# heyblackC/DFMIR

Measured on AMD Instinct MI355X. Metric: train-step image-pairs/sec (fwd+bwd): 2D 256x256 bs=16 and 3D 160^3 bs=1, higher is better.
Workload: dtype f32 (fp16x2-split MFMA, fp32 accumulate)

## Files before the change

### dfmir_amd/csrc/conv3x3s.hip

```cpp
#include "split_f16.h"

#ifndef PP_COMPUTE_PRIO
#define PP_COMPUTE_PRIO 1
#endif
#ifndef CS_COMPUTE_PRIO
#define CS_COMPUTE_PRIO 1
#endif
#ifndef CS_STORE_PRIO
#define CS_STORE_PRIO 0
#endif
typedef __bf16 bf16x8 __attribute__((ext_vector_type(8)));
typedef __bf16 bf16x2 __attribute__((ext_vector_type(2)));
typedef _Float16 f16x2 __attribute__((ext_vector_type(2)));
typedef float f32x2 __attribute__((ext_vector_type(2)));

__device__ __forceinline__ unsigned pk_bf16(float a, float b) {
  const f32x2 v = {a, b};
  return __builtin_bit_cast(unsigned, __builtin_convertvector(v, bf16x2));
}

template <int NSP>
__device__ __forceinline__ void split_pair(float x0, float x1, unsigned (&p)[NSP]) {
  if constexpr (NSP == 3) {
    p[0] = pk_bf16(x0, x1);
// ... 448 lines not shown
          if (k.act == 1) v = v > 0.f ? v : v * k.slope;
          else if (k.act == 2) v = tanhf(v);
          yb[(long long)co * HWo + q] = v;
        }
      }
    }
  }
}

constexpr int CS_TH = 8, CS_TW = 32, CS_PW = CS_TW + 2, CS_XP = 352;

__device__ __forceinline__ void cs_mma_chunk(const u32x4* __restrict__ Ab, const u32x4* __restrict__ Xb, int abase,
                                             const int (&pb)[2], f32x16 (&acc)[4],
                                             const __amdgpu_buffer_rsrc_t rw_, const unsigned (&wb)[9], u32x4 (&rw)[9],
                                             const __amdgpu_buffer_rsrc_t rx_, const unsigned (&gvo)[2][8],
                                             unsigned (&rx)[2][8]) {
  constexpr int SA = 9 * 2 * 64, SX = 2 * CS_XP;
  using P = Prod<2>;
  u32x4 a[2][2][2], b[2][2][2];
#define CS_LOAD(set_, t_)                                                                        \
  {                                                                                              \
    _Pragma("unroll") for (int i = 0; i < 2; ++i)                                                \
      _Pragma("unroll") for (int s = 0; s < 2; ++s) a[set_][i][s] = Ab[s * SA + (t_) * 128 + abase + i * 32]; \
    _Pragma("unroll") for (int j = 0; j < 2; ++j)                                                \
      _Pragma("unroll") for (int s = 0; s < 2; ++s) b[set_][j][s] = Xb[s * SX + pb[j] + ((t_) / 3) * CS_PW + (t_) % 3]; \
  }
  CS_LOAD(0, 0)
  __builtin_amdgcn_sched_barrier(0);
#pragma unroll
  for (int t = 0; t < 9; ++t) {
    if (t < 8) CS_LOAD((t + 1) & 1, t + 1)
#pragma unroll
    for (int q = 0; q < 3; ++q) {
      const int L = 3 * t + q;
      if (L < 9) rw[L] = __builtin_amdgcn_raw_buffer_load_b128(rw_, wb[L], 0, 0);
      else if (L < 25) rx[(L - 9) >> 3][(L - 9) & 7] = __builtin_amdgcn_raw_buffer_load_b32(rx_, gvo[(L - 9) >> 3][(L - 9) & 7], 0, 0);
    }
#pragma unroll
    for (int q = 0; q < P::N; ++q)
#pragma unroll
      for (int i = 0; i < 2; ++i)
#pragma unroll
        for (int j = 0; j < 2; ++j)
          acc[2 * i + j] = mma16<2>(b[t & 1][j][P::B[q]], a[t & 1][i][P::A[q]], acc[2 * i + j]);
    const int nds = t < 8 ? 8 : 0, nvm = (3 * t + 3 <= 25) ? 3 : (25 - 3 * t > 0 ? 25 - 3 * t : 0);
#pragma unroll
    for (int i = 0; i < 12; ++i) {
      __builtin_amdgcn_sched_group_barrier(0x008, 1, 0);
      if (i < nds) __builtin_amdgcn_sched_group_barrier(0x100, 1, 0);
      else if (i - nds < nvm) __builtin_amdgcn_sched_group_barrier(0x020, 1, 0);
    }
    __builtin_amdgcn_sched_barrier(0);
  }
#undef CS_LOAD
}

template <int CPG, int XP, int NW, int NS>
__device__ __forceinline__ void cs_mma_chunk_rr(const u32x4* __restrict__ Ab, const u32x4* __restrict__ Xb, int abase,
                                                int xb, f32x16 (&acc)[4],
                                                const __amdgpu_buffer_rsrc_t rw_, const unsigned (&wb)[NW], u32x4 (&rw)[NW],
                                                const __amdgpu_buffer_rsrc_t rx_, const unsigned (&gvo)[NS][8],
                                                unsigned (&rx)[NS][8]) {
  constexpr int SA = 9 * 2 * CPG, SX = 2 * XP;
  constexpr int NL = NW + 8 * NS;
  using P = Prod<2>;
  u32x4 a[9][2], xr[3][6][2];
#define CS_LDA(st_, s_) a[st_][s_] = Ab[(s_) * SA + (((st_) % 3) * 3 + (st_) / 3) * (2 * CPG) + abase];
#define CS_LDX(kx_, r_, s_) xr[kx_][r_][s_] = Xb[(s_) * SX + xb + (r_) * CS_PW + (kx_)];
#define CS_NEED(n_)                                                                              \
  {                                                                                              \
    constexpr int kx_ = (n_) / 3, ky_ = (n_) % 3;                                                \
    CS_LDA(n_, 1)                                                                                \
    if (ky_ == 0) { _Pragma("unroll") for (int r = 0; r < 4; ++r) CS_LDX(kx_, r, 0) }            \
    else CS_LDX(kx_, ky_ + 3, 0)                                                                 \
    CS_LDA(n_, 0)                                                                                \
    if (ky_ == 0) { _Pragma("unroll") for (int r = 0; r < 4; ++r) CS_LDX(kx_, r, 1) }            \
    else CS_LDX(kx_, ky_ + 3, 1)                                                                 \
  }
  CS_NEED(0)
  __builtin_amdgcn_sched_barrier(0);
#pragma unroll
  for (int st = 0; st < 9; ++st) {
    const int kx = st / 3, ky = st % 3;
    int nds = 0;
    if (st == 0) { CS_NEED(1) CS_NEED(2) nds = 8; }
    else if (st == 1) { CS_NEED(3) nds = 10; }
    else if (st == 2) { CS_NEED(4) nds = 4; }
    else if (st == 3) { CS_NEED(5) nds = 4; }
    else if (st == 4) { CS_NEED(6) nds = 10; }
    else if (st == 5) { CS_NEED(7) nds = 4; }
    else if (st == 6) { CS_NEED(8) nds = 4; }
    int L0, nvm;
    if (NL == 25) {
      L0 = st == 0 ? 0 : st == 1 ? 4 : st == 2 ? 6 : st == 3 ? 10 : st == 4 ? 14 : st == 5 ? 16 : st == 6 ? 20 : 24;
      nvm = (st == 1 || st == 4) ? 2 : (st == 7 ? 1 : (st == 8 ? 0 : 4));
    } else {
      const int lo = NL / 8, ex = NL % 8;
      L0 = st * lo + (st < ex ? st : ex);
      nvm = st < 8 ? lo + (st < ex ? 1 : 0) : 0;
    }
#pragma unroll
    for (int q = 0; q < (NL + 7) / 8; ++q) {
      const int L = L0 + q;
      if (q < nvm) {
        if (L < NW) rw[L] = __builtin_amdgcn_raw_buffer_load_b128(rw_, wb[L], 0, 0);
        else if (L < NL) rx[(L - NW) >> 3][(L - NW) & 7] = __builtin_amdgcn_raw_buffer_load_b32(rx_, gvo[(L - NW) >> 3][(L - NW) & 7], 0, 0);
      }
    }
#pragma unroll
    for (int q = 0; q < P::N; ++q)
#pragma unroll
      for (int j = 0; j < 4; ++j)
        acc[j] = mma16<2>(xr[kx][ky + j][P::B[q]], a[st][P::A[q]], acc[j]);
#pragma unroll
    for (int i = 0; i < 12; ++i) {
      __builtin_amdgcn_sched_group_barrier(0x008, 1, 0);
      if (i < nds) __builtin_amdgcn_sched_group_barrier(0x100, 1, 0);
      if (i >= 12 - nvm) __builtin_amdgcn_sched_group_barrier(0x020, 1, 0);
    }
    __builtin_amdgcn_sched_barrier(0);
  }
#undef CS_NEED
#undef CS_LDA
#undef CS_LDX
}

struct ConvCsP {
  int N, Cin, Cout, Hi, Wi, Ho, Wo, pad, pad_mode, act;
  float slope;
  int tiles_x, tiles_y;
  const float* res;
  const float* ring;
  int ring_rl;
  int xcd_pair;
  int dephase;
  int vec4;
};

#ifdef CS_TRACE
__device__ unsigned g_cs_trace[8 * 32 * 8 + 8];
extern "C" int dfmir_cs_trace_dump(unsigned* out) {
  return (int)hipMemcpyFromSymbol(out, HIP_SYMBOL(g_cs_trace), sizeof(unsigned) * (8 * 32 * 8 + 8));
}
#define TRC(slot_) { if (trace_blk && lane == 0) trc[((grp * 4 + wid) * 32 + (h & 31)) * 8 + (slot_)] = (unsigned)__builtin_readcyclecounter(); }
__device__ unsigned g_cs_wg[2048 * 6];
extern "C" int dfmir_cs_wg_dump(unsigned* out) {
  return (int)hipMemcpyFromSymbol(out, HIP_SYMBOL(g_cs_wg), sizeof(unsigned) * 2048 * 6);
}
#define WGT(slot_) { if (threadIdx.x == 0 && blockIdx.x < 2048 && blockIdx.y == 0) g_cs_wg[blockIdx.x * 6 + (slot_)] = (unsigned)wall_clock64(); }
#else
#define WGT(slot_)
#define TRC(slot_)
#endif
template <bool RR, int CPG, int TH>
__global__ __launch_bounds__(512, 1) void conv3x3_split_cs_k(const float* __restrict__ x, const u32x4* __restrict__ ws,
                                                             const float* __restrict__ bias, float* __restrict__ y,
                                                             ConvCsP k, SplitScale sc) {
  static_assert((CPG == 64 && TH == 8) || (RR && CPG == 32 && TH == 16), "tile forms");
  constexpr int CS_TH = TH;
  constexpr int NSP = 2, XP = (TH == 8 ? CS_XP : 640), NPOS = (CS_TH + 2) * CS_PW;
  constexpr int WUG = NSP * 9 * 2 * CPG;
  constexpr int NW = (WUG + 255) / 256;
  constexpr int NS = (NPOS + 255) / 256;
  __shared__ __attribute__((aligned(16))) u32x4 Wg[2][WUG];
  __shared__ __attribute__((aligned(16))) u32x4 Xs[2][NSP * 2 * XP];
  __shared__ float bs[2 * CPG];
#ifdef CS_TRACE
  __shared__ unsigned trc[8 * 32 * 8];
  const bool trace_blk = blockIdx.x == 300 && blockIdx.y == 0;
  const unsigned long long trc_t0 = __builtin_readcyclecounter(), trc_r0 = wall_clock64();
#endif

  const int grp = __builtin_amdgcn_readfirstlane((int)(threadIdx.x >> 8));
  const int tid = threadIdx.x & 255, lane = tid & 63, wid = tid >> 6;
  const int l31 = lane & 31, lhi = lane >> 5;
  const int HWo = k.Ho * k.Wo, HWi = k.Hi * k.Wi;
  if (k.dephase > 0 && blockIdx.y == 0 && blockIdx.x < 256) {
    const unsigned long long t0 = wall_clock64();
    const unsigned wait = blockIdx.x * (unsigned)k.dephase >> 8;
    while ((unsigned)(wall_clock64() - t0) < wait) __builtin_amdgcn_s_sleep(4);
  }
  WGT(0)
#ifdef CS_TRACE
  if (threadIdx.x == 0 && blockIdx.x < 2048 && blockIdx.y == 0) {
    g_cs_wg[blockIdx.x * 6 + 4] = __builtin_amdgcn_s_getreg(63492);
    g_cs_wg[blockIdx.x * 6 + 5] = __builtin_amdgcn_s_getreg(63508);
  }
#endif
  int bt = blockIdx.x, bm = blockIdx.y;
  if (k.xcd_pair == 1) { bm = (bt >> 3) & 1; bt = ((bt >> 4) << 3) + (bt & 7); }
  else if (k.xcd_pair >= 2) {
    const int ny = k.xcd_pair - 1, per = (int)(gridDim.x >> 3) / ny, j = bt >> 3;
    bm = j % ny;
    bt = (bt & 7) * per + j / ny;
  }
  const int tx = bt % k.tiles_x; bt /= k.tiles_x;
  const int ty = bt % k.tiles_y;
  const int n = bt / k.tiles_y;
  const int oy0 = ty * CS_TH, ox0 = tx * CS_TW;
  const int m0 = bm * (2 * CPG), m0g = m0 + CPG * grp;

  const int ex = scale_exp(reduce_absmax(sc.x_amax, sc.x_n, bs));
  __syncthreads();
  const int ew = (int)sc.w_trailer[1];
  const float xscale = pow2f(ex), oscale = pow2f(-ex), oscale2 = pow2f(-ew);

  constexpr unsigned OOB = 0x80000000u;
  unsigned gvo[NS][8];
#pragma unroll
  for (int s = 0; s < NS; ++s) {
    const int pos = tid + 256 * s;
    int off = -1;
    if (pos < NPOS) {
      const int r = pos / CS_PW, c = pos - r * CS_PW;
      off = halo_offset(oy0 - k.pad + r, ox0 - k.pad + c, k.Hi, k.Wi, k.pad_mode);
    }
#pragma unroll
    for (int c = 0; c < 8; ++c) gvo[s][c] = off < 0 ? OOB : (unsigned)(off + (8 * grp + c) * HWi) * 4u;
  }
  if (threadIdx.x < 2 * CPG) bs[threadIdx.x] = (bias && (m0 + (int)threadIdx.x) < k.Cout) ? bias[m0 + threadIdx.x] : 0.f;

  int pb[2];
#pragma unroll
  for (int j = 0; j < 2; ++j) pb[j] = lhi * XP + (2 * wid + j) * CS_PW + l31;
  const int rowgrp = CPG == 64 ? (wid >> 1) : wid;
  const int xb = lhi * XP + 4 * rowgrp * CS_PW + l31;
  const int abase = lhi * CPG + l31 + ((RR && CPG == 64) ? 32 * (wid & 1) : 0);

  f32x16 acc[4];
#pragma unroll
  for (int i = 0; i < 4; ++i)
#pragma unroll
    for (int r = 0; r < 16; ++r) acc[i][r] = 0.f;

  const float* xn = x + (long long)n * k.Cin * HWi;
  const int chunks8 = (k.Cin + 7) / 8, chunks = (k.Cin + 15) / 16;
  unsigned wb[NW];
#pragma unroll
  for (int j = 0; j < NW; ++j) {
    const int idx = tid + 256 * j;
    const int co = m0g + (idx % CPG), r = idx / CPG;
    const int half = r & 1, st = r >> 1;
    wb[j] = (idx < WUG && co < k.Cout) ? (unsigned)((half * NSP * 9 + st) * k.Cout + co) * 16u : OOB;
  }
  const int wunits8 = NSP * 9 * k.Cout;

  u32x4 rw[NW];
  unsigned rx[NS][8];
#define CS_GLOADW(c_)                                                                            \
  {                                                                                              \
    const int q_ = 2 * (c_);                                                                     \
    const int left_ = chunks8 - q_;                                                              \
    const __amdgpu_buffer_rsrc_t rw_ = __builtin_amdgcn_make_buffer_rsrc(                        \
        const_cast<u32x4*>(ws + (long long)q_ * wunits8), 0,                                     \
        left_ > 0 ? (unsigned)((left_ < 2 ? left_ : 2) * wunits8) * 16u : 0u, 0x00020000);       \
    _Pragma("unroll") for (int j = 0; j < NW; ++j) rw[j] = __builtin_amdgcn_raw_buffer_load_b128(rw_, wb[j], 0, 0); \
  }
#define CS_GLOADX(c_)                                                                            \
  {                                                                                              \
    const int c0_ = 16 * (c_);                                                                   \
    const int left_ = k.Cin - c0_;                                                               \
    const __amdgpu_buffer_rsrc_t rx_ = __builtin_amdgcn_make_buffer_rsrc(                        \
        const_cast<float*>(xn + (long long)c0_ * HWi), 0,                                        \
        left_ > 0 ? (unsigned)((left_ < 16 ? left_ : 16) * HWi) * 4u : 0u, 0x00020000);          \
    _Pragma("unroll") for (int s = 0; s < NS; ++s)                                               \
      _Pragma("unroll") for (int c = 0; c < 8; ++c)                                              \
        rx[s][c] = __builtin_amdgcn_raw_buffer_load_b32(rx_, gvo[s][c], 0, 0);                   \
  }
#define CS_LSTOREW()                                                                             \
  { _Pragma("unroll") for (int j = 0; j < NW; ++j) if (WUG % 256 == 0 || tid + 256 * j < WUG) Wg[grp][tid + 256 * j] = rw[j]; }
#define CS_LSTOREX(buf_)                                                                         \
  {                                                                                              \
    _Pragma("unroll") for (int s = 0; s < NS; ++s) {                                             \
      const int pos = tid + 256 * s;                                                             \
      if (pos < NPOS) {                                                                          \
        float v[8];                                                                              \
        _Pragma("unroll") for (int c = 0; c < 8; ++c) v[c] = __uint_as_float(rx[s][c]);          \
        CS_NORM_PROBE_OPS()                                                                      \
        u32x4 sp[NSP];                                                                           \
        split8_s<NSP>(v, xscale, sp);                                                                      \
        _Pragma("unroll") for (int q = 0; q < NSP; ++q) Xs[buf_][(q * 2 + grp) * XP + pos] = sp[q]; \
      }                                                                                          \
    }                                                                                            \
  }

#ifdef CS_NORM_PROBE
  const float np_r = fmaf(oscale2, 0.f, 1.f), np_m = oscale2 * 0.f, np_lo = fmaf(oscale2, 0.f, -3.0e38f);
#define CS_NORM_PROBE_OPS() _Pragma("unroll") for (int c = 0; c < 8; ++c) v[c] = fmaxf(fmaf(v[c], np_r, np_m), np_lo);
#else
#define CS_NORM_PROBE_OPS()
#endif
  CS_GLOADX(0);
  if (grp == 0) CS_GLOADW(0);
  CS_LSTOREX(0);
  if (grp == 0) CS_LSTOREW();
  if (grp == 1) { CS_GLOADW(0); CS_GLOADX(1); }
  __syncthreads();
  WGT(1)

  for (int h = 0; h < 2 * chunks; ++h) {
    const int c = h >> 1;
    TRC(0)
    if ((h & 1) == grp) {
      __builtin_amdgcn_s_setprio(CS_COMPUTE_PRIO);
      const int qw_ = 2 * (c + 1), lw_ = chunks8 - qw_;
      const __amdgpu_buffer_rsrc_t rwd = __builtin_amdgcn_make_buffer_rsrc(
          const_cast<u32x4*>(ws + (long long)qw_ * wunits8), 0,
          lw_ > 0 ? (unsigned)((lw_ < 2 ? lw_ : 2) * wunits8) * 16u : 0u, 0x00020000);
      const int cx_ = 16 * (c + 1 + grp), lx_ = k.Cin - cx_;
      const __amdgpu_buffer_rsrc_t rxd = __builtin_amdgcn_make_buffer_rsrc(
          const_cast<float*>(xn + (long long)cx_ * HWi), 0,
          lx_ > 0 ? (unsigned)((lx_ < 16 ? lx_ : 16) * HWi) * 4u : 0u, 0x00020000);
      if constexpr (RR) cs_mma_chunk_rr<CPG, XP, NW, NS>(Wg[grp], Xs[c & 1], abase, xb, acc, rwd, wb, rw, rxd, gvo, rx);
      else if constexpr (CPG == 64) cs_mma_chunk(Wg[grp], Xs[c & 1], abase, pb, acc, rwd, wb, rw, rxd, gvo, rx);
    } else {
      __builtin_amdgcn_s_setprio(CS_STORE_PRIO);
      {
#ifdef CS_TRACE
      __builtin_amdgcn_s_waitcnt(0x0f70);
      TRC(3)
#endif
#ifdef CS_TRACE
      CS_LSTOREW();
      TRC(4)
      if (c + 1 < chunks) CS_LSTOREX((c + 1) & 1);
#else
      if (grp == 0) {
        if (c + 1 < chunks) { CS_LSTOREW(); CS_LSTOREX((c + 1) & 1); }
      } else {
        CS_LSTOREW();
        if (c + 1 < chunks) CS_LSTOREX((c + 1) & 1);
      }
#endif
      }
    }
    TRC(1)
#ifndef CS_NO_EARLY_EPI
    if (h + 1 < 2 * chunks)
#endif
    __syncthreads();
    TRC(2)
  }
  WGT(2)
#ifdef CS_TRACE
  if (trace_blk) {
    __syncthreads();
    for (int i = threadIdx.x; i < 8 * 32 * 8; i += 512) g_cs_trace[i] = trc[i];
    if (threadIdx.x == 0) {
      const unsigned long long t1 = __builtin_readcyclecounter(), r1 = wall_clock64();
      g_cs_trace[2048] = (unsigned)trc_t0; g_cs_trace[2049] = (unsigned)t1;
      g_cs_trace[2050] = (unsigned)trc_r0; g_cs_trace[2051] = (unsigned)r1;
    }
  }
#endif
#undef CS_GLOADW
#undef CS_GLOADX
#undef CS_LSTOREW
#undef CS_LSTOREX
#undef CS_NORM_PROBE_OPS

  float* yb = y + (long long)n * k.Cout * HWo;
#pragma unroll
  for (int b = 0; b < 4; ++b) {
    const int i = CPG == 32 ? 0 : (RR ? (wid & 1) : (b >> 1));
    const int row = RR ? 4 * rowgrp + b : 2 * wid + (b & 1);
    const int oy = oy0 + row;
    const int cc = CPG * grp + i * 32 + l31, co = m0 + cc;
#ifdef CS_KO_EPI
    if (oy >= k.Ho || co >= k.Cout || acc[b][0] != 12345.678f) continue;
#else
    if (oy >= k.Ho || co >= k.Cout) continue;
#endif
    const float bv = bs[cc], osc = oscale * oscale2;
    const long long rowoff = (long long)co * HWo + (long long)oy * k.Wo;
    const float* rb = k.res ? k.res + (long long)n * k.Cout * HWo + rowoff : nullptr;
    const float* rg = k.ring ? k.ring + ((long long)n * 4 * k.Cout + co) * k.ring_rl : nullptr;
    const long long ss = (long long)k.Cout * k.ring_rl;
    const bool row_ring = rg != nullptr && (oy == 1 || oy == k.Ho - 2);
    float4 rv[4];
#pragma unroll
    for (int q = 0; q < 4; ++q) {
      rv[q] = make_float4(0.f, 0.f, 0.f, 0.f);
      const int ox = ox0 + 8 * q + 4 * lhi;
      if (rb && ox < k.Wo) {
        if (k.vec4) rv[q] = *reinterpret_cast<const float4*>(rb + ox);
        else {
          rv[q].x = rb[ox];
          if (ox + 1 < k.Wo) rv[q].y = rb[ox + 1];
          if (ox + 2 < k.Wo) rv[q].z = rb[ox + 2];
          if (ox + 3 < k.Wo) rv[q].w = rb[ox + 3];
        }
      }
    }
#pragma unroll
    for (int q = 0; q < 4; ++q) {
      const int ox = ox0 + 8 * q + 4 * lhi;
      if (ox >= k.Wo) continue;
      float v[4];
      const float r4[4] = {rv[q].x, rv[q].y, rv[q].z, rv[q].w};
#pragma unroll
      for (int e = 0; e < 4; ++e) {
        float t = acc[b][4 * q + e] * osc + bv;
        if (k.act == 1) t = t > 0.f ? t : t * k.slope;
        else if (k.act == 2) t = tanhf(t);
        v[e] = t + r4[e];
      }
      if (rg) {
#pragma unroll
        for (int e = 0; e < 4; ++e) {
          const int xx = ox + e;
          if (xx < k.Wo) {
            if (row_ring) {
              if (oy == 1) v[e] += rg[xx + 1] + (xx == 1 ? rg[0] : 0.f) + (xx == k.Wo - 2 ? rg[k.Wo + 1] : 0.f);
              if (oy == k.Ho - 2) v[e] += rg[ss + xx + 1] + (xx == 1 ? rg[ss] : 0.f) + (xx == k.Wo - 2 ? rg[ss + k.Wo + 1] : 0.f);
            }
            if (xx == 1) v[e] += rg[2 * ss + oy + 1];
            if (xx == k.Wo - 2) v[e] += rg[3 * ss + oy + 1];
          }
        }
      }
      float* yp = yb + rowoff + ox;
#ifdef CS_NT_STORE
      if (k.vec4) __builtin_nontemporal_store(f32x4{v[0], v[1], v[2], v[3]}, reinterpret_cast<f32x4*>(yp));
#else
      if (k.vec4) *reinterpret_cast<float4*>(yp) = make_float4(v[0], v[1], v[2], v[3]);
#endif
      else {
        yp[0] = v[0];
        if (ox + 1 < k.Wo) yp[1] = v[1];
        if (ox + 2 < k.Wo) yp[2] = v[2];
        if (ox + 3 < k.Wo) yp[3] = v[3];
      }
    }
  }
#ifdef CS_TRACE
  __builtin_amdgcn_s_waitcnt(0x0f70);
#endif
  WGT(3)
}

#ifdef DFMIR_BUILD_W1
#include "../../scripts/ubench/conv3x3_split_w1.inc"
#endif

static bool cs_plan(const DfConvGeom* g, int* th_out, int* tx_out, int* ty_out) {
  static DfOptFlag nocs_o{"DFMIR_CONV_NO_CS"};
  const bool use_cs = !nocs_o.get();
  static DfOptFlag plain_o{"DFMIR_CONV_CS_PLAIN"};
  const bool rr = !plain_o.get();
  if (!(df_split_mode() == 2 && use_cs && (g->Cout > 64 || rr))) return false;
  const int th = g->Cout > 64 ? 8 : 16;
  const int tx = (g->Wo + CS_TW - 1) / CS_TW, ty = (g->Ho + th - 1) / th;
  const double fill = (double)g->Ho * g->Wo / ((double)tx * CS_TW * ty * th);
  if (!((long long)g->N * tx * ty < (1LL << 31) && fill >= 0.85)) return false;
  *th_out = th; *tx_out = tx; *ty_out = ty;
  return true;
}
static bool split_fwd_geom_ok(const DfConvGeom* g) {
  if (!(g->KD == 1 && g->KH == 3 && g->KW == 3 && g->Di == 1 && g->Do == 1 && g->stride == 1 && g->dil == 1))
    return false;
  if (g->Cout <= 32 || g->Cin < 16 || g->ph != g->pw || g->pd != 0) return false;
  const int p = g->ph;
  if (!(p == 1 || (p == 2 && g->pad_mode == 0))) return false;
  if (g->Ho != g->Hi + 2 * p - 2 || g->Wo != g->Wi + 2 * p - 2) return false;
  const long long HWo = (long long)g->Ho * g->Wo;
  if (HWo >= (1LL << 30) || (long long)g->Hi * g->Wi >= (1LL << 30)) return false;
  if ((long long)((g->Cin + 7) / 8) * 27 * g->Cout * 16 >= (1LL << 31)) return false;
  if (worst_npos(g->Wo, (int)HWo, 128) > 399) return false;
  return true;
}
int df_conv3x3_split_res_ok(const DfConvGeom* g) {
  int th, tx, ty;
  return (df_split_mode() == 2 && split_fwd_geom_ok(g) && cs_plan(g, &th, &tx, &ty)) ? 1 : 0;
}
bool df_conv3x3_split_fwd_try(const DfConvGeom* g, const float* x, const float* x_amax, int x_n, const float* w_packed,
                              const float* bias, const float* res, const float* ring, int ring_rl, float* y,
                              hipStream_t st, int* rc) {
  const int mode = df_split_mode();
  if (mode == 0 || (mode == 2 && !(x_amax && x_n > 0))) return false;
  if (!split_fwd_geom_ok(g)) return false;
  const int p = g->ph;
  const long long HWo = (long long)g->Ho * g->Wo;
  Conv3P k{g->N, g->Cin, g->Cout, g->Hi, g->Wi, g->Ho, g->Wo, p, g->pad_mode, g->act, g->slope, 0};
  const u32x4* ws = reinterpret_cast<const u32x4*>(split_section(w_packed, g->Cin, g->Cout));
  const SplitScale sc{x_amax, x_n, split_trailer(w_packed, g->Cin, g->Cout, mode)};
  static DfOptFlag plain_o{"DFMIR_CONV_CS_PLAIN"};
  const bool rr = !plain_o.get();
  int th = 0, tlx = 0, tly = 0;
  if (mode == 2 && cs_plan(g, &th, &tlx, &tly)) {
    ConvCsP kc{g->N, g->Cin, g->Cout, g->Hi, g->Wi, g->Ho, g->Wo, p, g->pad_mode, g->act, g->slope, tlx, tly, res,
               ring, ring_rl, 0, 0, 0};
    kc.vec4 = (g->Wo % 4 == 0 && ((uintptr_t)y & 15) == 0 && ((uintptr_t)res & 15) == 0) ? 1 : 0;
    static DfOptInt dephase_o{"DFMIR_CS_DEPHASE", 0};
    const long long nb = (long long)g->N * tlx * tly;
    if (nb * ((g->Cout + 127) / 128) >= 512) kc.dephase = dephase_o.get();
    if (g->Cout > 64) {
      dim3 grid((unsigned)nb, (unsigned)((g->Cout + 127) / 128));
      static DfOptInt xcd_o{"DFMIR_CS_XCD_PAIR", 2};
  const int xcd_pair = xcd_o.get();
      if (xcd_pair && grid.y <= 2 && (nb & 7) == 0) {
        kc.xcd_pair = xcd_pair == 1 ? (grid.y == 2 ? 1 : 0) : (int)grid.y + 1;
        if (kc.xcd_pair) grid = dim3((unsigned)(grid.y * nb), 1u);
      }
#ifdef DFMIR_BUILD_W1
      static DfOptFlag w1_o{"DFMIR_CONV_W1"};
      if (w1_o.get() && rr && kc.vec4 && g->act != 2 && (g->Cin % 16) == 0 && (g->Ho % 16) == 0 && (g->Wo % 32) == 0) {
        ConvCsP kw = kc;
        kw.tiles_y = g->Ho / 16;
        const long long nbw = (long long)g->N * kw.tiles_x * kw.tiles_y;
        const unsigned gyw = (unsigned)((g->Cout + 127) / 128);
        kw.xcd_pair = 0;
        dim3 gw((unsigned)nbw, gyw);
        if ((nbw & 7) == 0 && gyw <= 2) { kw.xcd_pair = (int)gyw + 1; gw = dim3((unsigned)(gyw * nbw), 1u); }
        conv3x3_split_w1_k<0><<<gw, 256, 0, st>>>(x, ws, bias, y, kw, sc);
      } else
#endif
      if (rr) conv3x3_split_cs_k<true, 64, 8><<<grid, 512, 0, st>>>(x, ws, bias, y, kc, sc);
      else conv3x3_split_cs_k<false, 64, 8><<<grid, 512, 0, st>>>(x, ws, bias, y, kc, sc);
    } else {
      static DfOptInt xcd1_o{"DFMIR_CS_XCD_PAIR", 2};
    const int xcd1 = xcd1_o.get();
      if (xcd1 >= 2 && (nb & 7) == 0) kc.xcd_pair = 2;
      conv3x3_split_cs_k<true, 32, 16><<<dim3((unsigned)nb, 1u), 512, 0, st>>>(x, ws, bias, y, kc, sc);
    }
    hipError_t e = hipGetLastError();
    *rc = (e == hipSuccess) ? 0 : df_set_error((int)e, __FILE__, __LINE__);
    return true;
  }
  if (res || ring) { *rc = df_set_error((int)hipErrorInvalidValue, __FILE__, __LINE__); return true; }
  k.tiles_per_img = (int)((HWo + 255) / 256);
  const bool big = g->Cout > 64;
  dim3 grid((unsigned)(g->N * k.tiles_per_img), big ? (unsigned)((g->Cout + 127) / 128) : 1u);
  if (mode == 2) {
    if (big) conv3x3_split_pp_k<2, 400, 128><<<grid, 512, 0, st>>>(x, ws, bias, y, k, sc);
    else conv3x3_split_pp_k<2, 400, 64><<<grid, 512, 0, st>>>(x, ws, bias, y, k, sc);
  } else {
    if (big) conv3x3_split_pp_k<3, 400, 128><<<grid, 512, 0, st>>>(x, ws, bias, y, k, sc);
    else conv3x3_split_pp_k<3, 400, 64><<<grid, 512, 0, st>>>(x, ws, bias, y, k, sc);
  }
  hipError_t e = hipGetLastError();
  *rc = (e == hipSuccess) ? 0 : df_set_error((int)e, __FILE__, __LINE__);
  return true;
}

struct WS3P {
  int N, Cin, Cout, H, W, pad_mode;
  int runs_per_row, runs_per_img, runs_total, runs_per_block;
  const float* x_amax;
  const float* dy_amax;
  int x_n, dy_n;
  float* db;
  const float* dy_pmax;
  int swap;
  float* dbx;
  const float* fx;
};

template <int NSP, int BC>
__global__ __launch_bounds__(512, 1) void conv3x3_wgrad_split_k(const float* __restrict__ x,
                                                                const float* __restrict__ dy,
                                                                float* __restrict__ dwt, WS3P k) {
  using P = Prod<NSP>;
  constexpr int CT = 64, NWC = BC / 32, KS = 4 / NWC, NSTEP = 18 / KS;
  constexpr int XSLAB = 2 * CT;
  __shared__ __attribute__((aligned(16))) u32x4 Xc[NSP * 3 * 4 * XSLAB];
  __shared__ __attribute__((aligned(16))) u32x4 Dy[NSP * 2 * 2 * BC];
  __shared__ float bsum[BC];

  const int tid = threadIdx.x, lane = tid & 63, wid = tid >> 6;
  const bool want_db = k.db != nullptr && blockIdx.y == 0;
  if (tid < BC) bsum[tid] = 0.f;
  float bacc = 0.f;
  const int wc = wid % NWC, wi = (wid / NWC) & 1, kh = wid / (2 * NWC);
  const int l31 = lane & 31, lhi = lane >> 5;
  const int HW = k.H * k.W;
  const int ci0 = blockIdx.y * CT, co0 = blockIdx.z * BC;
  const int run_beg = blockIdx.x * k.runs_per_block;
  int run_end = run_beg + k.runs_per_block;
  if (run_end > k.runs_total) run_end = k.runs_total;

  float xscale = 1.f, dscale = 1.f, oscale = 1.f, oscale2 = 1.f;
  if (NSP == 2) {
    __shared__ float red[17];
    const int ex = scale_exp(reduce_absmax(k.x_amax, k.x_n, red));
    __syncthreads();
    const int ed = scale_exp(reduce_absmax(k.dy_amax, k.dy_n, red));
    xscale = pow2f(ex); dscale = pow2f(ed); oscale = pow2f(-ex); oscale2 = pow2f(-ed);
  }

  const int xc = tid & 63, xu = (tid >> 6) & 1, xr = tid >> 7;
  const int dc = tid % BC, du = (tid / BC) & 1, dk = (tid / (2 * BC)) & 1;
  const bool dload = tid < 4 * BC;
  const unsigned hw4 = (unsigned)HW * 4u;
  constexpr unsigned OOB = 0x80000000u;

  f32x16 acc[9];
#pragma unroll
  for (int t = 0; t < 9; ++t)
#pragma unroll
    for (int r = 0; r < 16; ++r) acc[t][r] = 0.f;

  u32x4 rxa, rxb, rda, rdb;
  unsigned rxl, rxr;

#define WS_GLOAD(run_)                                                                           \
  {                                                                                              \
    const int n_ = (run_) / k.runs_per_img;                                                      \
    const int q_ = (run_) - n_ * k.runs_per_img;                                                 \
    const int yp_ = q_ / k.runs_per_row, xs_ = q_ - yp_ * k.runs_per_row;                        \
    const int y0_ = 2 * yp_, x0_ = 16 * xs_ + 8 * xu;                                            \
    const __amdgpu_buffer_rsrc_t bx_ = __builtin_amdgcn_make_buffer_rsrc(                        \
        const_cast<float*>(x + (long long)n_ * k.Cin * HW), 0, (unsigned)(k.Cin * HW) * 4u, 0x00020000); \
    const __amdgpu_buffer_rsrc_t bd_ = __builtin_amdgcn_make_buffer_rsrc(                        \
        const_cast<float*>(dy + (long long)n_ * k.Cout * HW), 0, (unsigned)(k.Cout * HW) * 4u, 0x00020000); \
    const bool cok_ = ci0 + xc < k.Cin;                                                          \
    const unsigned cb_ = (unsigned)(ci0 + xc) * hw4;                                             \
     \
                                             \
    int ry_ = y0_ - 1 + xr;                                                                      \
    bool rok_ = (unsigned)ry_ < (unsigned)k.H;                                                   \
    if (k.pad_mode == 1) { ry_ = ry_ < 0 ? -ry_ : (ry_ >= k.H ? 2 * (k.H - 1) - ry_ : ry_); rok_ = true; } \
    const int rb_ = ry_ * k.W;                                                                   \
    const bool lin_ = x0_ > 0, rin_ = x0_ + 8 < k.W;                                             \
    const int ol_ = rb_ + (lin_ ? x0_ - 1 : 1), or_ = rb_ + (rin_ ? x0_ + 8 : k.W - 2);          \
    const bool lok_ = rok_ && cok_ && (lin_ || k.pad_mode == 1), rrok_ = rok_ && cok_ && (rin_ || k.pad_mode == 1); \
    const unsigned xb_ = (rok_ && cok_) ? cb_ + (unsigned)(rb_ + x0_) * 4u : OOB;                \
    rxa = __builtin_amdgcn_raw_buffer_load_b128(bx_, xb_, 0, 0);                                 \
    rxb = __builtin_amdgcn_raw_buffer_load_b128(bx_, xb_ == OOB ? OOB : xb_ + 16u, 0, 0);        \
    rxl = __builtin_amdgcn_raw_buffer_load_b32(bx_, lok_ ? cb_ + (unsigned)ol_ * 4u : OOB, 0, 0); \
    rxr = __builtin_amdgcn_raw_buffer_load_b32(bx_, rrok_ ? cb_ + (unsigned)or_ * 4u : OOB, 0, 0); \
    const unsigned db_ = (co0 + dc >= k.Cout || !dload) ? OOB                                    \
        : (unsigned)(co0 + dc) * hw4 + (unsigned)((y0_ + dk) * k.W + 16 * xs_ + 8 * du) * 4u;    \
    rda = __builtin_amdgcn_raw_buffer_load_b128(bd_, db_, 0, 0);                                 \
    rdb = __builtin_amdgcn_raw_buffer_load_b128(bd_, db_ == OOB ? OOB : db_ + 16u, 0, 0);        \
  }
#define WS_LSTORE()                                                                              \
  {                                                                                              \
    float r[10];                                                                                 \
    r[0] = __uint_as_float(rxl); r[9] = __uint_as_float(rxr);                                    \
    _Pragma("unroll") for (int e = 0; e < 4; ++e) { r[1 + e] = __uint_as_float(rxa[e]); r[5 + e] = __uint_as_float(rxb[e]); } \
    unsigned pa[5][NSP], pb[4][NSP];                                                             \
    _Pragma("unroll") for (int i = 0; i < 5; ++i) split_pair_s<NSP>(r[2 * i], r[2 * i + 1], xscale, pa[i]); \
    if (NSP == 2) {             \
      _Pragma("unroll") for (int i = 0; i < 4; ++i)                                              \
        _Pragma("unroll") for (int s = 0; s < NSP; ++s) pb[i][s] = __builtin_amdgcn_alignbit(pa[i + 1][s], pa[i][s], 16); \
    } else {                                                                                     \
      _Pragma("unroll") for (int i = 0; i < 4; ++i) split_pair<NSP>(r[2 * i + 1], r[2 * i + 2], pb[i]); \
    }                                                                                            \
    _Pragma("unroll") for (int s = 0; s < NSP; ++s) {                                            \
      u32x4* dst = Xc + ((s * 3 * 4 + xr) * 2 + xu) * CT + xc;                                   \
      dst[0] = u32x4{pa[0][s], pa[1][s], pa[2][s], pa[3][s]};                                    \
      dst[4 * XSLAB] = u32x4{pb[0][s], pb[1][s], pb[2][s], pb[3][s]};                            \
      dst[8 * XSLAB] = u32x4{pa[1][s], pa[2][s], pa[3][s], pa[4][s]};                            \
    }                                                                                            \
    float v[8];                                                                                  \
    _Pragma("unroll") for (int e = 0; e < 4; ++e) { v[e] = __uint_as_float(rda[e]); v[4 + e] = __uint_as_float(rdb[e]); } \
    bacc += ((v[0] + v[1]) + (v[2] + v[3])) + ((v[4] + v[5]) + (v[6] + v[7]));    \
    u32x4 sp[NSP];                                                                               \
    split8_s<NSP>(v, dscale, sp);                                                                \
    if (dload) { _Pragma("unroll") for (int s = 0; s < NSP; ++s) Dy[((s * 2 + dk) * 2 + du) * BC + dc] = sp[s]; } \
  }

  if (run_beg < run_end) {
    WS_GLOAD(run_beg);
    WS_LSTORE();
  }
  __syncthreads();

  const int abase = lhi * CT + wi * 32 + l31 + (KS == 2 ? kh * XSLAB : 0);
  const int bbase = lhi * BC + wc * 32 + l31 + (KS == 2 ? kh * 2 * BC : 0);
  for (int run = run_beg; run < run_end; ++run) {
    const bool more = (run + 1) < run_end;
    if (more) WS_GLOAD(run + 1);
    u32x4 b[NSP], a[2][NSP];
#define WS_LOADA(set_, step_)                                                                    \
  _Pragma("unroll") for (int s = 0; s < NSP; ++s)                                                \
// ... 552 lines not shown
```

Before: 210.1.

## Add multi-tile persistent loop to split conv3x3 kernel behind env option

Adds a template parameter T so each workgroup walks several horizontal output tiles in sequence. The channel-chunk pipeline runs continuously across tile boundaries, with the epilogue issued mid-loop and the accumulators reset between tiles. This amortises per-workgroup setup (absmax reduction, bias load, pipeline fill) for shallow-Cin layers. It also moves the first global loads ahead of the scale reduction. The new path is off by default (DFMIR_CS_TILES=1), so only that load reordering changes the default path, at the cost of more code complexity and register pressure.

After: 205.7. 0.979x the previous value.

```diff
diff --git a/dfmir_amd/csrc/conv3x3s.hip b/dfmir_amd/csrc/conv3x3s.hip
--- a/dfmir_amd/csrc/conv3x3s.hip
+++ b/dfmir_amd/csrc/conv3x3s.hip
@@ -624,11 +624,12 @@
 #define WGT(slot_)
 #define TRC(slot_)
 #endif
-template <bool RR, int CPG, int TH>
+template <bool RR, int CPG, int TH, int T = 1>
 __global__ __launch_bounds__(512, 1) void conv3x3_split_cs_k(const float* __restrict__ x, const u32x4* __restrict__ ws,
                                                              const float* __restrict__ bias, float* __restrict__ y,
                                                              ConvCsP k, SplitScale sc) {
   static_assert((CPG == 64 && TH == 8) || (RR && CPG == 32 && TH == 16), "tile forms");
+  static_assert(T >= 1, "tiles per workgroup");
   constexpr int CS_TH = TH;
   constexpr int NSP = 2, XP = (TH == 8 ? CS_XP : 640), NPOS = (CS_TH + 2) * CS_PW;
   constexpr int WUG = NSP * 9 * 2 * CPG;
@@ -666,31 +667,32 @@
     bm = j % ny;
     bt = (bt & 7) * per + j / ny;
   }
-  const int tx = bt % k.tiles_x; bt /= k.tiles_x;
+  const int tgx = (k.tiles_x + T - 1) / T;
+  const int tx = (bt % tgx) * T; bt /= tgx;
   const int ty = bt % k.tiles_y;
   const int n = bt / k.tiles_y;
   const int oy0 = ty * CS_TH, ox0 = tx * CS_TW;
   const int m0 = bm * (2 * CPG), m0g = m0 + CPG * grp;
-
-  const int ex = scale_exp(reduce_absmax(sc.x_amax, sc.x_n, bs));
-  __syncthreads();
-  const int ew = (int)sc.w_trailer[1];
-  const float xscale = pow2f(ex), oscale = pow2f(-ex), oscale2 = pow2f(-ew);
+  const int ntl = T == 1 ? 1 : (k.tiles_x - tx < T ? k.tiles_x - tx : T);
 
   constexpr unsigned OOB = 0x80000000u;
   unsigned gvo[NS][8];
-#pragma unroll
-  for (int s = 0; s < NS; ++s) {
-    const int pos = tid + 256 * s;
-    int off = -1;
-    if (pos < NPOS) {
-      const int r = pos / CS_PW, c = pos - r * CS_PW;
-      off = halo_offset(oy0 - k.pad + r, ox0 - k.pad + c, k.Hi, k.Wi, k.pad_mode);
-    }
-#pragma unroll
-    for (int c = 0; c < 8; ++c) gvo[s][c] = off < 0 ? OOB : (unsigned)(off + (8 * grp + c) * HWi) * 4u;
-  }
-  if (threadIdx.x < 2 * CPG) bs[threadIdx.x] = (bias && (m0 + (int)threadIdx.x) < k.Cout) ? bias[m0 + threadIdx.x] : 0.f;
+  auto set_gvo = [&](int ox0_) {
+    int tid_ = tid;
+    if constexpr (T > 1) asm volatile("" : "+v"(tid_));
+#pragma unroll
+    for (int s = 0; s < NS; ++s) {
+      const int pos = tid_ + 256 * s;
+      int off = -1;
+      if (pos < NPOS) {
+        const int r = pos / CS_PW, c = pos - r * CS_PW;
+        off = halo_offset(oy0 - k.pad + r, ox0_ - k.pad + c, k.Hi, k.Wi, k.pad_mode);
+      }
+#pragma unroll
+      for (int c = 0; c < 8; ++c) gvo[s][c] = off < 0 ? OOB : (unsigned)(off + (8 * grp + c) * HWi) * 4u;
+    }
+  };
+  set_gvo(ox0);
 
   int pb[2];
 #pragma unroll
@@ -719,19 +721,19 @@
 
   u32x4 rw[NW];
   unsigned rx[NS][8];
-#define CS_GLOADW(c_)                                                                            \
+#define CS_GLOADW(c_, live_)                                                                     \
   {                                                                                              \
     const int q_ = 2 * (c_);                                                                     \
-    const int left_ = chunks8 - q_;                                                              \
+    const int left_ = (live_) ? chunks8 - q_ : 0;                                                \
     const __amdgpu_buffer_rsrc_t rw_ = __builtin_amdgcn_make_buffer_rsrc(                        \
         const_cast<u32x4*>(ws + (long long)q_ * wunits8), 0,                                     \
         left_ > 0 ? (unsigned)((left_ < 2 ? left_ : 2) * wunits8) * 16u : 0u, 0x00020000);       \
     _Pragma("unroll") for (int j = 0; j < NW; ++j) rw[j] = __builtin_amdgcn_raw_buffer_load_b128(rw_, wb[j], 0, 0); \
   }
-#define CS_GLOADX(c_)                                                                            \
+#define CS_GLOADX(c_, live_)                                                                     \
   {                                                                                              \
     const int c0_ = 16 * (c_);                                                                   \
-    const int left_ = k.Cin - c0_;                                                               \
+    const int left_ = (live_) ? k.Cin - c0_ : 0;                                                 \
     const __amdgpu_buffer_rsrc_t rx_ = __builtin_amdgcn_make_buffer_rsrc(                        \
         const_cast<float*>(xn + (long long)c0_ * HWi), 0,                                        \
         left_ > 0 ? (unsigned)((left_ < 16 ? left_ : 16) * HWi) * 4u : 0u, 0x00020000);          \
@@ -762,24 +764,128 @@
 #else
 #define CS_NORM_PROBE_OPS()
 #endif
-  CS_GLOADX(0);
-  if (grp == 0) CS_GLOADW(0);
+  const int G = ntl * chunks;
+  int cm = 0, tl = 0;
+  auto at = [&](int d, int& cc_, int& tt_) {
+    cc_ = cm + d; tt_ = tl;
+    if constexpr (T > 1) { while (cc_ >= chunks) { cc_ -= chunks; ++tt_; } }
+  };
+  int gt = 0;
+  auto aim_gvo = [&](int tt_) {
+    if (tt_ != gt && tt_ < ntl) { gt = tt_; set_gvo(ox0 + tt_ * CS_TW); }
+  };
+
+  CS_GLOADX(0, true);
+  if (grp == 0) CS_GLOADW(0, true);
+  const int ex = scale_exp(reduce_absmax(sc.x_amax, sc.x_n, bs));
+  __syncthreads();
+  const int ew = (int)sc.w_trailer[1];
+  const float xscale = pow2f(ex), oscale = pow2f(-ex), oscale2 = pow2f(-ew);
+  if (threadIdx.x < 2 * CPG) bs[threadIdx.x] = (bias && (m0 + (int)threadIdx.x) < k.Cout) ? bias[m0 + threadIdx.x] : 0.f;
+  int c1_ = 1, t1_ = 0;
+  if constexpr (T > 1) { at(1, c1_, t1_); aim_gvo(t1_); }
   CS_LSTOREX(0);
   if (grp == 0) CS_LSTOREW();
-  if (grp == 1) { CS_GLOADW(0); CS_GLOADX(1); }
+  if (grp == 1) { CS_GLOADW(0, true); CS_GLOADX(c1_, t1_ < ntl); }
   __syncthreads();
   WGT(1)
 
-  for (int h = 0; h < 2 * chunks; ++h) {
+  auto epilogue = [&](const int ox0_) {
+  int tid_ = tid;
+  if constexpr (T > 1) asm volatile("" : "+v"(tid_));
+  const int wid_ = tid_ >> 6, l31_ = tid_ & 31, lhi_ = (tid_ >> 5) & 1;
+  const int rowgrp_ = CPG == 64 ? (wid_ >> 1) : wid_;
+  float* yb = y + (long long)n * k.Cout * HWo;
+#pragma unroll
+  for (int b = 0; b < 4; ++b) {
+    const int i = CPG == 32 ? 0 : (RR ? (wid_ & 1) : (b >> 1));
+    const int row = RR ? 4 * rowgrp_ + b : 2 * wid_ + (b & 1);
+    const int oy = oy0 + row;
+    const int cc = CPG * grp + i * 32 + l31_, co = m0 + cc;
+#ifdef CS_KO_EPI
+    if (oy >= k.Ho || co >= k.Cout || acc[b][0] != 12345.678f) continue;
+#else
+    if (oy >= k.Ho || co >= k.Cout) continue;
+#endif
+    const float bv = bs[cc], osc = oscale * oscale2;
+    const long long rowoff = (long long)co * HWo + (long long)oy * k.Wo;
+    const float* rb = k.res ? k.res + (long long)n * k.Cout * HWo + rowoff : nullptr;
+    const float* rg = k.ring ? k.ring + ((long long)n * 4 * k.Cout + co) * k.ring_rl : nullptr;
+    const long long ss = (long long)k.Cout * k.ring_rl;
+    const bool row_ring = rg != nullptr && (oy == 1 || oy == k.Ho - 2);
+    float4 rv[4];
+#pragma unroll
+    for (int q = 0; q < 4; ++q) {
+      rv[q] = make_float4(0.f, 0.f, 0.f, 0.f);
+      const int ox = ox0_ + 8 * q + 4 * lhi_;
+      if (rb && ox < k.Wo) {
+        if (k.vec4) rv[q] = *reinterpret_cast<const float4*>(rb + ox);
+        else {
+          rv[q].x = rb[ox];
+          if (ox + 1 < k.Wo) rv[q].y = rb[ox + 1];
+          if (ox + 2 < k.Wo) rv[q].z = rb[ox + 2];
+          if (ox + 3 < k.Wo) rv[q].w = rb[ox + 3];
+        }
+      }
+    }
+#pragma unroll
+    for (int q = 0; q < 4; ++q) {
+      const int ox = ox0_ + 8 * q + 4 * lhi_;
+      if (ox >= k.Wo) continue;
+      float v[4];
+      const float r4[4] = {rv[q].x, rv[q].y, rv[q].z, rv[q].w};
+#pragma unroll
+      for (int e = 0; e < 4; ++e) {
+        float t = acc[b][4 * q + e] * osc + bv;
+        if (k.act == 1) t = t > 0.f ? t : t * k.slope;
+        else if (k.act == 2) t = tanhf(t);
+        v[e] = t + r4[e];
+      }
+      if (rg) {
+#pragma unroll
+        for (int e = 0; e < 4; ++e) {
+          const int xx = ox + e;
+          if (xx < k.Wo) {
+            if (row_ring) {
+              if (oy == 1) v[e] += rg[xx + 1] + (xx == 1 ? rg[0] : 0.f) + (xx == k.Wo - 2 ? rg[k.Wo + 1] : 0.f);
+              if (oy == k.Ho - 2) v[e] += rg[ss + xx + 1] + (xx == 1 ? rg[ss] : 0.f) + (xx == k.Wo - 2 ? rg[ss + k.Wo + 1] : 0.f);
+            }
+            if (xx == 1) v[e] += rg[2 * ss + oy + 1];
+            if (xx == k.Wo - 2) v[e] += rg[3 * ss + oy + 1];
+          }
+        }
+      }
+      float* yp = yb + rowoff + ox;
+#ifdef CS_NT_STORE
+      if (k.vec4) __builtin_nontemporal_store(f32x4{v[0], v[1], v[2], v[3]}, reinterpret_cast<f32x4*>(yp));
+#else
+      if (k.vec4) *reinterpret_cast<float4*>(yp) = make_float4(v[0], v[1], v[2], v[3]);
+#endif
+      else {
+        yp[0] = v[0];
+        if (ox + 1 < k.Wo) yp[1] = v[1];
+        if (ox + 2 < k.Wo) yp[2] = v[2];
+        if (ox + 3 < k.Wo) yp[3] = v[3];
+      }
+    }
+  }
+  };
+
+  for (int h = 0; h < 2 * G + (T > 1 ? 1 : 0); ++h) {
     const int c = h >> 1;
+    if constexpr (T == 1) cm = c;
+    if (T > 1 && h == 2 * G && grp == 0) break;
     TRC(0)
     if ((h & 1) == grp) {
       __builtin_amdgcn_s_setprio(CS_COMPUTE_PRIO);
-      const int qw_ = 2 * (c + 1), lw_ = chunks8 - qw_;
+      int cw_, tw_, cx2_, tx2_;
+      at(1, cw_, tw_);
+      at(1 + grp, cx2_, tx2_);
+      const int qw_ = 2 * cw_, lw_ = (T == 1 || tw_ < ntl) ? chunks8 - qw_ : 0;
       const __amdgpu_buffer_rsrc_t rwd = __builtin_amdgcn_make_buffer_rsrc(
           const_cast<u32x4*>(ws + (long long)qw_ * wunits8), 0,
           lw_ > 0 ? (unsigned)((lw_ < 2 ? lw_ : 2) * wunits8) * 16u : 0u, 0x00020000);
-      const int cx_ = 16 * (c + 1 + grp), lx_ = k.Cin - cx_;
+      const int cx_ = 16 * cx2_, lx_ = (T == 1 || tx2_ < ntl) ? k.Cin - cx_ : 0;
       const __amdgpu_buffer_rsrc_t rxd = __builtin_amdgcn_make_buffer_rsrc(
           const_cast<float*>(xn + (long long)cx_ * HWi), 0,
           lx_ > 0 ? (unsigned)((lx_ < 16 ? lx_ : 16) * HWi) * 4u : 0u, 0x00020000);
@@ -793,22 +899,37 @@
       TRC(3)
 #endif
 #ifdef CS_TRACE
-      CS_LSTOREW();
+      if (T == 1 || c < G) CS_LSTOREW();
       TRC(4)
-      if (c + 1 < chunks) CS_LSTOREX((c + 1) & 1);
+      if (c + 1 < G) CS_LSTOREX((c + 1) & 1);
 #else
       if (grp == 0) {
-        if (c + 1 < chunks) { CS_LSTOREW(); CS_LSTOREX((c + 1) & 1); }
+        if (c + 1 < G) { CS_LSTOREW(); CS_LSTOREX((c + 1) & 1); }
       } else {
-        CS_LSTOREW();
-        if (c + 1 < chunks) CS_LSTOREX((c + 1) & 1);
-      }
-#endif
+        if (T == 1 || c < G) CS_LSTOREW();
+        if (c + 1 < G) CS_LSTOREX((c + 1) & 1);
+      }
+#endif
+      }
+      if constexpr (T > 1) {
+        if (grp == 0 ? cm == chunks - 1 : (cm == 0 && c > 0)) {
+          epilogue(ox0 + (tl - grp) * CS_TW);
+#pragma unroll
+          for (int i = 0; i < 4; ++i)
+#pragma unroll
+            for (int r = 0; r < 16; ++r) acc[i][r] = 0.f;
+        }
+        int c2_, t2_;
+        at(2, c2_, t2_);
+        aim_gvo(t2_);
       }
     }
     TRC(1)
+    if constexpr (T > 1) {
+      if (h & 1) { if (++cm == chunks) { cm = 0; ++tl; } }
+    }
 #ifndef CS_NO_EARLY_EPI
-    if (h + 1 < 2 * chunks)
+    if (h + 1 < 2 * G)
 #endif
     __syncthreads();
     TRC(2)
@@ -831,80 +952,7 @@
 #undef CS_LSTOREX
 #undef CS_NORM_PROBE_OPS
 
-  float* yb = y + (long long)n * k.Cout * HWo;
-#pragma unroll
-  for (int b = 0; b < 4; ++b) {
-    const int i = CPG == 32 ? 0 : (RR ? (wid & 1) : (b >> 1));
-    const int row = RR ? 4 * rowgrp + b : 2 * wid + (b & 1);
-    const int oy = oy0 + row;
-    const int cc = CPG * grp + i * 32 + l31, co = m0 + cc;
-#ifdef CS_KO_EPI
-    if (oy >= k.Ho || co >= k.Cout || acc[b][0] != 12345.678f) continue;
-#else
-    if (oy >= k.Ho || co >= k.Cout) continue;
-#endif
-    const float bv = bs[cc], osc = oscale * oscale2;
-    const long long rowoff = (long long)co * HWo + (long long)oy * k.Wo;
-    const float* rb = k.res ? k.res + (long long)n * k.Cout * HWo + rowoff : nullptr;
-    const float* rg = k.ring ? k.ring + ((long long)n * 4 * k.Cout + co) * k.ring_rl : nullptr;
-    const long long ss = (long long)k.Cout * k.ring_rl;
-    const bool row_ring = rg != nullptr && (oy == 1 || oy == k.Ho - 2);
-    float4 rv[4];
-#pragma unroll
-    for (int q = 0; q < 4; ++q) {
-      rv[q] = make_float4(0.f, 0.f, 0.f, 0.f);
-      const int ox = ox0 + 8 * q + 4 * lhi;
-      if (rb && ox < k.Wo) {
-        if (k.vec4) rv[q] = *reinterpret_cast<const float4*>(rb + ox);
-        else {
-          rv[q].x = rb[ox];
-          if (ox + 1 < k.Wo) rv[q].y = rb[ox + 1];
-          if (ox + 2 < k.Wo) rv[q].z = rb[ox + 2];
-          if (ox + 3 < k.Wo) rv[q].w = rb[ox + 3];
-        }
-      }
-    }
-#pragma unroll
-    for (int q = 0; q < 4; ++q) {
-      const int ox = ox0 + 8 * q + 4 * lhi;
-      if (ox >= k.Wo) continue;
-      float v[4];
-      const float r4[4] = {rv[q].x, rv[q].y, rv[q].z, rv[q].w};
-#pragma unroll
-      for (int e = 0; e < 4; ++e) {
-        float t = acc[b][4 * q + e] * osc + bv;
-        if (k.act == 1) t = t > 0.f ? t : t * k.slope;
-        else if (k.act == 2) t = tanhf(t);
-        v[e] = t + r4[e];
-      }
-      if (rg) {
-#pragma unroll
-        for (int e = 0; e < 4; ++e) {
-          const int xx = ox + e;
-          if (xx < k.Wo) {
-            if (row_ring) {
-              if (oy == 1) v[e] += rg[xx + 1] + (xx == 1 ? rg[0] : 0.f) + (xx == k.Wo - 2 ? rg[k.Wo + 1] : 0.f);
-              if (oy == k.Ho - 2) v[e] += rg[ss + xx + 1] + (xx == 1 ? rg[ss] : 0.f) + (xx == k.Wo - 2 ? rg[ss + k.Wo + 1] : 0.f);
-            }
-            if (xx == 1) v[e] += rg[2 * ss + oy + 1];
-            if (xx == k.Wo - 2) v[e] += rg[3 * ss + oy + 1];
-          }
-        }
-      }
-      float* yp = yb + rowoff + ox;
-#ifdef CS_NT_STORE
-      if (k.vec4) __builtin_nontemporal_store(f32x4{v[0], v[1], v[2], v[3]}, reinterpret_cast<f32x4*>(yp));
-#else
-      if (k.vec4) *reinterpret_cast<float4*>(yp) = make_float4(v[0], v[1], v[2], v[3]);
-#endif
-      else {
-        yp[0] = v[0];
-        if (ox + 1 < k.Wo) yp[1] = v[1];
-        if (ox + 2 < k.Wo) yp[2] = v[2];
-        if (ox + 3 < k.Wo) yp[3] = v[3];
-      }
-    }
-  }
+  if constexpr (T == 1) epilogue(ox0);
 #ifdef CS_TRACE
   __builtin_amdgcn_s_waitcnt(0x0f70);
 #endif
@@ -927,6 +975,12 @@
   if (!((long long)g->N * tx * ty < (1LL << 31) && fill >= 0.85)) return false;
   *th_out = th; *tx_out = tx; *ty_out = ty;
   return true;
+}
+static int cs_tiles(const DfConvGeom* g, int tiles_x) {
+  static DfOptInt tiles_o{"DFMIR_CS_TILES", 1};
+  const int want = tiles_o.get();
+  const int chunks = (g->Cin + 15) / 16;
+  return ((want == 2 || want == 4) && chunks <= 8 && tiles_x >= 2) ? want : 1;
 }
 static bool split_fwd_geom_ok(const DfConvGeom* g) {
   if (!(g->KD == 1 && g->KH == 3 && g->KW == 3 && g->Di == 1 && g->Do == 1 && g->stride == 1 && g->dil == 1))
@@ -964,7 +1018,8 @@
                ring, ring_rl, 0, 0, 0};
     kc.vec4 = (g->Wo % 4 == 0 && ((uintptr_t)y & 15) == 0 && ((uintptr_t)res & 15) == 0) ? 1 : 0;
     static DfOptInt dephase_o{"DFMIR_CS_DEPHASE", 0};
-    const long long nb = (long long)g->N * tlx * tly;
+    const int mt = cs_tiles(g, tlx);
+    const long long nb = (long long)g->N * ((tlx + mt - 1) / mt) * tly;
     if (nb * ((g->Cout + 127) / 128) >= 512) kc.dephase = dephase_o.get();
     if (g->Cout > 64) {
       dim3 grid((unsigned)nb, (unsigned)((g->Cout + 127) / 128));
@@ -987,13 +1042,20 @@
         conv3x3_split_w1_k<0><<<gw, 256, 0, st>>>(x, ws, bias, y, kw, sc);
       } else
 #endif
-      if (rr) conv3x3_split_cs_k<true, 64, 8><<<grid, 512, 0, st>>>(x, ws, bias, y, kc, sc);
+      if (rr && mt == 4) conv3x3_split_cs_k<true, 64, 8, 4><<<grid, 512, 0, st>>>(x, ws, bias, y, kc, sc);
+      else if (rr && mt == 2) conv3x3_split_cs_k<true, 64, 8, 2><<<grid, 512, 0, st>>>(x, ws, bias, y, kc, sc);
+      else if (rr) conv3x3_split_cs_k<true, 64, 8><<<grid, 512, 0, st>>>(x, ws, bias, y, kc, sc);
+      else if (mt == 4) conv3x3_split_cs_k<false, 64, 8, 4><<<grid, 512, 0, st>>>(x, ws, bias, y, kc, sc);
+      else if (mt == 2) conv3x3_split_cs_k<false, 64, 8, 2><<<grid, 512, 0, st>>>(x, ws, bias, y, kc, sc);
       else conv3x3_split_cs_k<false, 64, 8><<<grid, 512, 0, st>>>(x, ws, bias, y, kc, sc);
     } else {
       static DfOptInt xcd1_o{"DFMIR_CS_XCD_PAIR", 2};
     const int xcd1 = xcd1_o.get();
       if (xcd1 >= 2 && (nb & 7) == 0) kc.xcd_pair = 2;
-      conv3x3_split_cs_k<true, 32, 16><<<dim3((unsigned)nb, 1u), 512, 0, st>>>(x, ws, bias, y, kc, sc);
+      const dim3 grid1((unsigned)nb, 1u);
+      if (mt == 4) conv3x3_split_cs_k<true, 32, 16, 4><<<grid1, 512, 0, st>>>(x, ws, bias, y, kc, sc);
+      else if (mt == 2) conv3x3_split_cs_k<true, 32, 16, 2><<<grid1, 512, 0, st>>>(x, ws, bias, y, kc, sc);
+      else conv3x3_split_cs_k<true, 32, 16><<<grid1, 512, 0, st>>>(x, ws, bias, y, kc, sc);
     }
     hipError_t e = hipGetLastError();
     *rc = (e == hipSuccess) ? 0 : df_set_error((int)e, __FILE__, __LINE__);
```
